# ali-vilab/VGen

Measured on AMD Instinct MI355X. Metric: denoise_steps_per_sec, higher is better.
Workload: dtype fp16

## Files before the change

include/vgen_hip.h:

```cpp
#ifndef VGEN_HIP_H
#define VGEN_HIP_H

#include <stddef.h>
#include <stdint.h>

#ifdef __cplusplus
extern "C" {
#endif

#define VGEN_ABI_VERSION 7

enum { VGEN_BF16 = 0, VGEN_F16 = 1, VGEN_F32 = 2 };

enum {
  VGEN_E_BADARG = -1,
  VGEN_E_UNSUPPORTED = -2,
  VGEN_E_WORKSPACE = -3
};

int vgen_version(void);
const char* vgen_last_error(void);

size_t vgen_groupnorm_ws_bytes(int64_t nb, int64_t S);
int vgen_groupnorm(const float* x1, int32_t C1, const float* x2, int32_t C2,
                   int64_t nb, int64_t S, int32_t groups, float eps,
                   const float* gamma, const float* beta, int32_t silu,
                   void* y, void* raw, int32_t raw_split, int32_t dtype,
                   float* ws, size_t ws_bytes, void* stream);

int vgen_groupnorm_cs(const float* x1, int32_t C1, const float* cs1,
                      const float* x2, int32_t C2, const float* cs2,
                      int64_t nb, int64_t S, int32_t groups, float eps,
                      const float* gamma, const float* beta, int32_t silu,
                      void* y, void* raw, int32_t raw_split, int32_t dtype,
                      float* ws, size_t ws_bytes, void* stream);

int vgen_embed_tokens(const int64_t* tokens, int64_t rows, int32_t L, int32_t d, int32_t vocab,
                      const float* table, const float* pos, float* out, void* stream);

int vgen_layernorm(const float* x, int64_t M, int32_t d, float eps,
                   const float* gamma, const float* beta,
                   void* y, int32_t dtype, void* stream);

enum { VGEN_TAP_LINEAR = 0, VGEN_TAP_CONV3X3 = 1, VGEN_TAP_TEMPORAL3 = 2 };
enum { VGEN_EPI_NONE = 0, VGEN_EPI_GEGLU = 1 };

typedef struct vgen_tapgemm_args {
  int64_t M;
  int32_t N;
  int32_t dtype;
  const void* A;
  int64_t lda;
  int32_t C1;
  int32_t taps;
  int32_t mode;
  int32_t Hi, Wi, Ho, Wo, stride, pad_t, pad_l, ups;
  int32_t F;
  int64_t S;
  const void* A2;
  int64_t lda2;
  int32_t C2;
  const void* W;
  int64_t ldw;
  const float* bias;
  const float* rowbias;
  int64_t rowbias_ld;
  int64_t rows_per_rb;
  const float* residual;
  int64_t ldr;
  void* out;
  int64_t ldo;
  int32_t out_dtype;
  int32_t epilogue;
  void* ws;
  size_t ws_bytes;
  int32_t crop_t;
  float* colstats;
  int32_t dualw;
  int32_t split_out;
} vgen_tapgemm_args;

size_t vgen_tapgemm_ws_bytes(const vgen_tapgemm_args* args);
int vgen_tapgemm(const vgen_tapgemm_args* args, void* stream);

int vgen_tapgemm_query_plan(const vgen_tapgemm_args* args, int32_t* out3);
int vgen_tapgemm_set_plans(const int64_t* rows, int32_t n);

typedef struct vgen_attn_args {
  const void* q;
  const void* k;
  const void* v;
  void* out;
  int32_t dtype;
  int32_t heads;
  int32_t nq, nk;
  int64_t nbatch;
  int64_t inner;
  int64_t q_rs, q_bo, q_bi;
  int64_t k_rs, k_bo, k_bi;
  int64_t v_rs, v_bo, v_bi;
  int64_t o_rs, o_bo, o_bi;
  float scale;
  int32_t causal;
} vgen_attn_args;

int vgen_attention(const vgen_attn_args* args, void* stream);

int vgen_attention_d80(const vgen_attn_args* args, void* stream);

int vgen_softmax_rows(const float* S, int64_t rows, int32_t cols, int64_t lds, float scale,
                      void* P, int64_t ldp, int32_t dtype, void* stream);


int vgen_act_cast(const float* x, void* y, int64_t n, int32_t act, int32_t dtype, void* stream);

int vgen_cast_split(const float* x, int64_t M, int32_t C, int64_t ldx, void* out, int64_t ldo, int32_t lo_off,
                    int32_t dtype, void* stream);

int vgen_timestep_embedding(const float* t, int32_t B, int32_t dim, void* out, int32_t dtype,
                            void* stream);

int vgen_linear_f32(const float* x, int32_t n, int32_t K, const float* W, const float* bias, int32_t N,
                    int32_t act_in, const float* add, float* out, void* stream);

int vgen_im2col3x3_small(const float* src, int64_t nimg, int32_t Fi, int32_t Cin, int32_t H,
                         int32_t W, int64_t s_bo, int64_t s_fi, int64_t s_c, int64_t s_y,
                         int64_t s_x, void* out, int32_t Kpad, int32_t dtype, int32_t split, void* stream);

int vgen_pointwise_small(const float* src, int64_t nimg, int32_t Fi, int32_t Cin, int32_t H,
                         int32_t W, int64_t s_bo, int64_t s_fi, int64_t s_c, int64_t s_y,
                         int64_t s_x, const float* Wm, const float* b, int32_t Cout, float* dst,
                         int64_t d_bo, int64_t d_fi, int64_t d_c, int64_t d_y, int64_t d_x,
                         void* stream);

int vgen_cfg_ddim_step(const float* xt, const float* y, const float* u, const float* noise,
                       const float* coef, float guide, int32_t use_guide, int32_t mean_type,
                       int64_t B, int64_t per_b, float* xt_1, float* x0_out, void* stream);

int vgen_cfg_ddim_step_units(const float* xt, int64_t xt_bstride, const float* y, const float* u,
                             const float* noise, const float* coef, const int64_t* t_idx, float guide,
                             int32_t use_guide, int32_t mean_type, int64_t B, int64_t per_b, float* xt_1,
                             float* x0_out, float* rep, int32_t nrep, int64_t rep_gstride,
                             int64_t rep_bstride, void* stream);

int vgen_gaussian_sample(const float* moments, const float* noise, int64_t nimg, int32_t zc,
                         int64_t HW, float scale, float* z, void* stream);

int vgen_lowfreq_filter(const float* x, int64_t nimg, int32_t H, int32_t W, int32_t C, float scale,
                        float* y, float* ws, size_t ws_bytes, void* stream);
int vgen_scale_channels(float* x, int64_t M, int32_t C, int32_t c0, int32_t c1, float s, void* stream);

int vgen_patchify(const float* x, int64_t B, int32_t C, int32_t H, int32_t W, int32_t P, int32_t Kpad, int32_t cls,
                  void* out, int32_t dtype, void* stream);

int vgen_conv3x3_small(const float* x, int64_t n, int32_t Cin, int32_t H, int32_t W, const float* w,
                       const float* b, int32_t Cout, int32_t stride, int32_t act, float* y, void* stream);
int vgen_adaptive_avgpool2d(const float* x, int64_t planes, int32_t H, int32_t W, int32_t Ho, int32_t Wo,
                            float* y, void* stream);
int vgen_frame_transformer(const float* x, int64_t B, int32_t F, int32_t d, int64_t HW, int32_t heads,
                           int32_t dim_head, int32_t hidden, const float* ln_w, const float* ln_b,
                           const float* wqkv, const float* wout, const float* bout, const float* w1,
                           const float* b1, const float* w2, const float* b2, float* y, int32_t last,
                           float out_scale, int32_t accumulate, void* stream);

int vgen_frames_u8(const float* x, int64_t rows, int32_t C, int64_t ldx, const float* mean,
                   const float* stdv, void* out, void* stream);

int vgen_adapter(const float* x, int64_t ldx, int64_t M, int32_t d, int32_t h, int32_t hp, const void* Wd,
                 const void* Wu, const float* bu, const float* hb, int64_t ldhb, int64_t rows_per_hb, float* out,
// ... 22 lines not shown
```

vgen_amd/build.py:

```python
from __future__ import annotations

import os
import shutil
import subprocess
import sys
from concurrent.futures import ThreadPoolExecutor

HERE = os.path.dirname(os.path.abspath(__file__))
CSRC = os.path.join(HERE, "csrc")
OBJ = os.path.join(CSRC, "_obj")
LIB = os.path.join(HERE, "libvgen_hip.so")
SOURCES = ["cabi.cpp", "tapgemm.hip", "panelgemm.hip", "norms.hip", "attention.hip", "misc.hip", "stems.hip", "adapter.hip"]
HEADERS = [os.path.join(CSRC, "common.h"), os.path.join(CSRC, "tapgemm_plans.inc"),
           os.path.join(HERE, "..", "include", "vgen_hip.h")]
FLAGS = ["--offload-arch=gfx950", "-O3", "-std=c++17", "-fPIC", "-Wall", "-Wno-unused-function", "-Wno-inline-asm",
         "-x", "hip"]


def _hipcc() -> str:
    for cand in (os.environ.get("HIPCC"), shutil.which("hipcc"), "/opt/rocm/bin/hipcc"):
        if cand and os.path.exists(cand):
            return cand
    raise RuntimeError("hipcc not found (need ROCm to build libvgen_hip.so)")


def _stale(target: str, deps) -> bool:
    if not os.path.exists(target):
        return True
    t = os.path.getmtime(target)
    return any(os.path.getmtime(d) > t for d in deps)


TUNING_LIB = os.path.join(HERE, "libvgen_hip_tuning.so")
HOST_LIB = os.path.join(HERE, "libvgen_host.so")
HOST_FLAGS = ["-O3", "-std=c++17", "-fPIC", "-shared", "-ffp-contract=off", "-Wall", "-pthread"]
HOST_ARCH = (["-march=x86-64-v3"], ["-mavx2", "-mf16c"])


def build_host(force: bool = False, verbose: bool = False) -> str:
    src = os.path.join(CSRC, "host_round.cpp")
    if force or _stale(HOST_LIB, [src]):
        gxx = os.environ.get("CXX") or shutil.which("g++") or shutil.which("c++")
        if not gxx:
            raise RuntimeError("g++ not found (need a host C++ compiler to build libvgen_host.so)")
        err = None
        for arch in HOST_ARCH:
            cmd = [gxx] + HOST_FLAGS + arch + [src, "-o", HOST_LIB]
            if verbose:
                print(" ".join(cmd), flush=True)
            r = subprocess.run(cmd, capture_output=True, text=True)
            if r.returncode == 0:
                err = None
                break
            err = "build failed: %s\n%s\n%s" % (" ".join(cmd), r.stdout, r.stderr)
        if err:
            raise RuntimeError(err)
    return HOST_LIB


def build_host_optional(force: bool = False, verbose: bool = False):
    try:
        return build_host(force=force, verbose=verbose)
    except (RuntimeError, OSError) as exc:
        import warnings
        warnings.warn(f"libvgen_host.so not built ({str(exc).splitlines()[0]}); vgen_amd.calibrate uses its torch loop")
        return None


def build(force: bool = False, verbose: bool = False, tuning: bool = False, variant: str = "", defines=()) -> str:
    if tuning:
        variant, defines = "tuning", tuple(defines) + ("VGEN_TUNING",)
    obj_dir = OBJ + ("_" + variant if variant else "")
    lib_path = os.path.join(HERE, f"libvgen_hip_{variant}.so") if variant else LIB
    flags = FLAGS + ["-D" + d for d in defines]
    os.makedirs(obj_dir, exist_ok=True)
    hipcc = _hipcc()
    jobs = []
    objs = []
    for src in SOURCES:
        s = os.path.join(CSRC, src)
        o = os.path.join(obj_dir, os.path.splitext(src)[0] + ".o")
        objs.append(o)
        if force or _stale(o, [s] + HEADERS):
            jobs.append([hipcc] + flags + ["-c", s, "-o", o])

    def run(cmd):
        if verbose:
            print(" ".join(cmd), flush=True)
        r = subprocess.run(cmd, capture_output=True, text=True)
        if r.returncode != 0:
            raise RuntimeError("build failed: %s\n%s\n%s" % (" ".join(cmd), r.stdout, r.stderr))
        return r

    if jobs:
        with ThreadPoolExecutor(max_workers=min(len(jobs), os.cpu_count() or 2)) as ex:
# ... 12 lines not shown
```

vgen_amd/csrc/tapgemm.hip:

```cpp
#include "common.h"
#include <stdio.h>
#include <stdlib.h>
#include <type_traits>

int vgen_panel_bn(const vgen_tapgemm_args& a);
int vgen_panel_launch(const vgen_tapgemm_args& a, hipStream_t s);

namespace {

struct RowState {
  int base;
  int a;
  int b;
};

constexpr int INVALID = -(1 << 24);

constexpr int ZERO_BYTES = 262144;
__device__ __attribute__((aligned(128))) unsigned char g_zeros[ZERO_BYTES];

typedef const __attribute__((address_space(1))) void* gptr_t;
typedef __attribute__((address_space(3))) void* lptr_t;


__device__ __forceinline__ void glds16(const void* src, unsigned char* lds_wave_base) {
  __builtin_amdgcn_global_load_lds((gptr_t)src, (lptr_t)lds_wave_base, 16, 0, 0);
}


template <int N>
__device__ __forceinline__ void wait_vmcnt() {
  asm volatile("s_waitcnt vmcnt(%0)" ::"n"(N) : "memory");
}

template <int CPR>
__device__ __forceinline__ int swz_key(int row) {
  if constexpr (CPR == 8) {
    return row & 7;
  } else {
    const int q = (row >> 2) & 3;
    return (4 - q) & 3;
  }
}

#ifdef VGEN_TUNING
#define VGEN_ABLATE_ARG(x) (x)
#else
#define VGEN_ABLATE_ARG(x) 0
#endif

template <typename T, int BM, int BN, int BK, int WM, int WN, int STAGES, bool PP, bool DW>
__global__ __launch_bounds__(WM* WN * 64, (WM * WN == 4) ? 2 : 1) void tapgemm_kernel(
    const vgen_tapgemm_args p, const int splitk, float* __restrict__ ws, const int ablate_arg, const int stagger,
    const int first_round) {
  static_assert(!PP || (WM * WN == 8 && STAGES == 3), "ping-pong needs 8 waves and a 3-stage ring");
  static_assert(!DW || (PP && BK == 64), "dual-W K-steps are built on the ping-pong schedule, 64-element K-tiles");
  const int ablate = VGEN_ABLATE_ARG(ablate_arg);
  constexpr int WPA = DW ? 2 : 1;
  constexpr int NT = WM * WN * 64;
  constexpr int ROW_BYTES = BK * 2;
  constexpr int CPR = ROW_BYTES / 16;
  constexpr int RPI = 64 / CPR;
  constexpr int RPP = NT / CPR;
  constexpr int KS = BK / 32;
  constexpr int WTM = BM / WM, WTN = BN / WN;
  constexpr int MF = WTM / 16, NF = WTN / 16;
  constexpr int RA = BM / RPP;
  constexpr int RBF = BN / RPP;
  constexpr int RBT = BN % RPP;
  constexpr int STAGE_BYTES = (BM + BN) * ROW_BYTES;
  constexpr int LPT = RA + RBF;
  static_assert(BM % RPP == 0 && RBT % RPI == 0, "tile rows must split into whole DMA instructions");

  extern __shared__ __attribute__((aligned(16))) unsigned char smem[];

  const int tid = threadIdx.x;
  const int lane = tid & 63;
  const int wave = __builtin_amdgcn_readfirstlane(tid >> 6);
  const int wm = wave / WN;
  const int wn = wave % WN;
  const int lr = lane & 15;
  const int lq = lane >> 4;
  const bool w_tail = RBT > 0 && wave * RPI < RBT;

  if (stagger > 0 && (int)(blockIdx.x + gridDim.x * blockIdx.y) < first_round && wave == 0) {
    const unsigned hw = __builtin_amdgcn_s_getreg((3 << 11) | ((WM * WN == 8 ? 8 : 0) << 6) | 4);
    if (hw & 1u)
      for (int i = 0; i < stagger; ++i) __builtin_amdgcn_s_sleep(16);
  }
// ... 792 lines not shown
    splitk = 1;
#ifdef VGEN_TUNING
  const char* ab = getenv("VGEN_TAPGEMM_ABLATE");
  const int ablate = ab ? atoi(ab) : 0;
#else
  const int ablate = 0;
#endif
  constexpr int BPC = (WM * WN == 4) ? 2 : 1;
  const int cus = vgen_device_cus();
  int stagger = 0;
  {
    int pct = BPC == 1 ? STAGGER_PCT_PP : STAGGER_PCT_DUAL, min_rounds = STAGGER_MIN_ROUNDS;
#ifdef VGEN_TUNING
    if (const char* e = getenv("VGEN_TAPGEMM_STAGGER")) {
      int a1 = 0, a2 = 0, a3 = min_rounds;
      if (sscanf(e, "%d,%d,%d", &a1, &a2, &a3) >= 2) {
        pct = BPC == 1 ? a1 : a2;
        min_rounds = a3;
      }
    }
#endif
    const int64_t blocks = grid * splitk;
    const double rounds = (double)blocks / ((double)cus * BPC);
    if (pct > 0 && rounds >= (double)min_rounds) {
      const int KT = a.taps * (a.C1 / 64) + a.C2 / 64;
      const int kts = (KT + splitk - 1) / splitk;
      const double tile_us = kts * (a.dualw ? 1.6 : 1.0) * (BM == 256 ? (BPC == 1 ? 0.0060 * BN : 0.0150 * BN) : 0.0050 * BN) + 7.0;
      stagger = (int)(tile_us * pct / 100.0 * 2400.0 / 1024.0 + 0.5);
    }
  }
  hipLaunchKernelGGL((tapgemm_kernel<T, BM, BN, BK, WM, WN, STAGES, PP, DW>), dim3((unsigned)grid, (unsigned)splitk),
                     dim3(WM * WN * 64), lds, stream, a, splitk, (float*)a.ws, ablate, stagger, cus * BPC);
  int rc = vgen_check_launch("tapgemm");
  if (rc || splitk == 1) return rc;
  const int n_out = a.epilogue == VGEN_EPI_GEGLU ? a.N / 2 : a.N;
  const int64_t threads = a.M * (n_out / 4);
  hipLaunchKernelGGL((splitk_reduce_kernel<T>), dim3((unsigned)((threads + 255) / 256)), dim3(256), 0,
                     stream, a, splitk, (const float*)a.ws);
  return vgen_check_launch("tapgemm(splitk reduce)");
}

int panel_bn(const vgen_tapgemm_args& a) {
#ifdef VGEN_TUNING
  if (env_int("VGEN_TAPGEMM_PANEL", 1) == 0) return 0;
#endif
  return vgen_panel_bn(a);
}

Plan full_plan(const vgen_tapgemm_args& a) {
  bool tabled = false;
  const Plan pl = make_plan(a, &tabled);
  if (!tabled)
    if (const int bn = panel_bn(a)) return Plan{SHAPE_PANEL, bn, 1};
  return pl;
}

template <typename T>
int dispatch(const vgen_tapgemm_args& a, hipStream_t s) {
  const Plan pl = full_plan(a);
  if (pl.shape == SHAPE_PANEL) return vgen_panel_launch(a, s);
  if (a.dualw) {
    if (pl.shape == SHAPE_PP128) {
      switch (pl.bn) {
        case 128: return launch<T, 128, 128, 64, 4, 2, 3, true, true>(a, pl.splitk, s);
        case 160: return launch<T, 128, 160, 64, 4, 2, 3, true, true>(a, pl.splitk, s);
        default: return launch<T, 128, 64, 64, 4, 2, 3, true, true>(a, pl.splitk, s);
      }
    }
    switch (pl.bn) {
      case 128: return launch<T, 256, 128, 64, 4, 2, 3, true, true>(a, pl.splitk, s);
      case 160: return launch<T, 256, 160, 64, 4, 2, 3, true, true>(a, pl.splitk, s);
      default: return launch<T, 256, 64, 64, 4, 2, 3, true, true>(a, pl.splitk, s);
    }
  }
  if (pl.shape == SHAPE_PP256) return launch<T, 256, 256, 32, 4, 2, 3, true>(a, pl.splitk, s);
  if (pl.shape == SHAPE_Q128) {
    switch (pl.bn) {
      case 128: return launch<T, 128, 128, 32, 2, 2, 3, false>(a, pl.splitk, s);
      case 160: return launch<T, 128, 160, 32, 2, 2, 3, false>(a, pl.splitk, s);
      default: return launch<T, 128, 64, 32, 2, 2, 3, false>(a, pl.splitk, s);
    }
  }
  if (pl.shape == SHAPE_PP) {
    switch (pl.bn) {
      case 128: return launch<T, 256, 128, 64, 4, 2, 3, true>(a, pl.splitk, s);
      case 160: return launch<T, 256, 160, 64, 4, 2, 3, true>(a, pl.splitk, s);
      default: return launch<T, 256, 64, 64, 4, 2, 3, true>(a, pl.splitk, s);
    }
  }
  if (pl.shape == SHAPE_PP128) {
    switch (pl.bn) {
      case 128: return launch<T, 128, 128, 64, 4, 2, 3, true>(a, pl.splitk, s);
      case 160: return launch<T, 128, 160, 64, 4, 2, 3, true>(a, pl.splitk, s);
      default: return launch<T, 128, 64, 64, 4, 2, 3, true>(a, pl.splitk, s);
    }
  }
  switch (pl.bn) {
    case 128: return launch<T, 256, 128, 32, 2, 2, 3, false>(a, pl.splitk, s);
    case 160: return launch<T, 256, 160, 32, 2, 2, 3, false>(a, pl.splitk, s);
    default: return launch<T, 256, 64, 32, 2, 2, 3, false>(a, pl.splitk, s);
  }
}

}

extern "C" int vgen_tapgemm_query_plan(const vgen_tapgemm_args* args, int32_t* out3) {
  if (!args || !out3 || args->N <= 0 || args->M <= 0 || args->C1 <= 0 || args->C1 % 64 || args->C2 % 64) return VGEN_E_BADARG;
  const Plan pl = full_plan(*args);
  out3[0] = pl.shape;
  out3[1] = pl.bn;
  out3[2] = pl.splitk;
  return 0;
}

extern "C" int vgen_tapgemm_set_plans(const int64_t* rows, int32_t n) {
  if (n < 0) {
    free(g_plans);
    g_plans = nullptr;
    g_nplans = -1;
    return 0;
  }
  if (n > 0 && !rows) return VGEN_E_BADARG;
  PlanEntry* t = (PlanEntry*)malloc(sizeof(PlanEntry) * (n > 0 ? n : 1));
  if (!t) return VGEN_E_BADARG;
  for (int i = 0; i < n; ++i) {
    const int64_t* r = rows + 12 * i;
    t[i] = PlanEntry{(int)r[0], r[1], (int)r[2], (int)r[3], (int)r[4], (int)r[5], (int)r[6], (int)r[7], (int)r[8],
                     (int)r[9], (int)r[10], (int)r[11]};
  }
  free(g_plans);
  g_plans = t;
  g_nplans = n;
  return 0;
}

extern "C" size_t vgen_tapgemm_ws_bytes(const vgen_tapgemm_args* args) {
  if (!args || args->N <= 0 || args->M <= 0 || args->C1 <= 0 || args->C1 % 64 || args->C2 % 64) return 0;
  const int s = full_plan(*args).splitk;
  return s > 1 ? (size_t)s * args->M * args->N * sizeof(float) : 0;
}

extern "C" int vgen_tapgemm(const vgen_tapgemm_args* args, void* stream) {
  if (!args) {
    vgen_set_error("tapgemm: null args");
    return VGEN_E_BADARG;
  }
  const vgen_tapgemm_args& a = *args;
  VGEN_REQUIRE(a.dtype == VGEN_BF16 || a.dtype == VGEN_F16, "tapgemm: dtype must be bf16/f16");
  VGEN_REQUIRE(a.M >= 0 && a.N > 0, "tapgemm: bad M/N");
  VGEN_REQUIRE(a.C1 > 0 && a.C1 % 64 == 0 && a.C2 >= 0 && a.C2 % 64 == 0,
               "tapgemm: C1=%d / C2=%d must be multiples of 64", a.C1, a.C2);
  VGEN_REQUIRE(a.dualw == 0 || a.dualw == 1, "tapgemm: dualw must be 0 or 1");
  VGEN_REQUIRE(a.lda % 8 == 0 && (a.C2 == 0 || a.lda2 % 8 == 0) && a.ldw % 8 == 0 &&
                   (a.ldw == 0 || a.ldw >= ((int64_t)a.taps * a.C1 + a.C2) * (a.dualw ? 2 : 1)),
               "tapgemm: lda/lda2/ldw must be multiples of 8 (ldw >= K, 2 K with dualw)");
  VGEN_REQUIRE(vgen_aligned16(a.A) && vgen_aligned16(a.W) && vgen_aligned16(a.out) &&
                   (a.C2 == 0 || (a.A2 && vgen_aligned16(a.A2))),
               "tapgemm: pointers must be 16-byte aligned");
  VGEN_REQUIRE(a.bias == nullptr || vgen_aligned16(a.bias), "tapgemm: bias alignment");
  VGEN_REQUIRE(a.residual == nullptr || vgen_aligned16(a.residual), "tapgemm: residual alignment");
  VGEN_REQUIRE(a.rowbias == nullptr || (vgen_aligned16(a.rowbias) && a.rows_per_rb > 0),
               "tapgemm: rowbias alignment / rows_per_rb");
  VGEN_REQUIRE(a.out_dtype == VGEN_F32 || a.out_dtype == a.dtype, "tapgemm: out_dtype");
  VGEN_REQUIRE(a.ws == nullptr || vgen_aligned16(a.ws), "tapgemm: workspace alignment");
  switch (a.mode) {
    case VGEN_TAP_LINEAR:
      VGEN_REQUIRE(a.taps == 1, "tapgemm: linear mode needs taps == 1");
      break;
    case VGEN_TAP_CONV3X3:
      VGEN_REQUIRE(a.taps == 9 && a.Hi > 0 && a.Wi > 0 && a.Ho > 0 && a.Wo > 0 &&
                       (a.stride == 1 || a.stride == 2) && (a.ups == 0 || a.ups == 1) && a.crop_t >= 0 &&
                       (a.crop_t == 0 || a.ups == 1),
                   "tapgemm: bad conv3x3 geometry");
      VGEN_REQUIRE(a.M % ((int64_t)a.Ho * a.Wo) == 0, "tapgemm: M not a multiple of Ho*Wo");
      VGEN_REQUIRE((a.M / ((int64_t)a.Ho * a.Wo)) * a.Hi * a.Wi < (1LL << 31),
                   "tapgemm: source row index overflows int32");
      break;
    case VGEN_TAP_TEMPORAL3:
      VGEN_REQUIRE(a.taps == 3 && a.F > 0 && a.S > 0 && a.M % (a.S * a.F) == 0,
                   "tapgemm: bad temporal geometry");
      break;
    default:
      vgen_set_error("tapgemm: unknown mode %d", a.mode);
      return VGEN_E_BADARG;
  }
  VGEN_REQUIRE(a.M + 256 < (1LL << 31), "tapgemm: M overflows int32 row index");
  VGEN_REQUIRE(a.lda >= 0 && a.lda < (1LL << 30) && a.lda2 >= 0 && a.lda2 < (1LL << 30),
               "tapgemm: lda / lda2 must be in [0, 2^30)");
  VGEN_REQUIRE(((int64_t)a.taps * a.C1 + a.C2) * (a.dualw ? 4 : 2) <= ZERO_BYTES - 128,
               "tapgemm: K = %lld too long (<= 131008; <= 65504 with dualw)",
               (long long)((int64_t)a.taps * a.C1 + a.C2));
  if (a.epilogue == VGEN_EPI_GEGLU) {
    VGEN_REQUIRE(a.N % 64 == 0 && a.rowbias == nullptr && (a.ldo % 4 == 0) &&
                     (a.residual == nullptr || a.ldr % 4 == 0),
                 "tapgemm: GEGLU needs N %% 64 == 0, no rowbias, ldo/ldr %% 4 == 0");
// ... 21 lines not shown
```

vgen_amd/lib.py:

```python
from __future__ import annotations

import ctypes as C
import os

HERE = os.path.dirname(os.path.abspath(__file__))
LIB_PATH = os.environ.get("VGEN_HIP_LIB") or os.path.join(HERE, "libvgen_hip.so")

VGEN_BF16, VGEN_F16, VGEN_F32 = 0, 1, 2
TAP_LINEAR, TAP_CONV3X3, TAP_TEMPORAL3 = 0, 1, 2
EPI_NONE, EPI_GEGLU = 0, 1
ABI_VERSION = 7


class VgenHipError(RuntimeError):
    pass


class TapGemmArgs(C.Structure):
    _fields_ = [
        ("M", C.c_int64), ("N", C.c_int32), ("dtype", C.c_int32),
        ("A", C.c_void_p), ("lda", C.c_int64), ("C1", C.c_int32), ("taps", C.c_int32),
        ("mode", C.c_int32),
        ("Hi", C.c_int32), ("Wi", C.c_int32), ("Ho", C.c_int32), ("Wo", C.c_int32),
        ("stride", C.c_int32), ("pad_t", C.c_int32), ("pad_l", C.c_int32), ("ups", C.c_int32),
        ("F", C.c_int32), ("S", C.c_int64),
        ("A2", C.c_void_p), ("lda2", C.c_int64), ("C2", C.c_int32),
        ("W", C.c_void_p), ("ldw", C.c_int64),
        ("bias", C.c_void_p), ("rowbias", C.c_void_p), ("rowbias_ld", C.c_int64),
        ("rows_per_rb", C.c_int64), ("residual", C.c_void_p), ("ldr", C.c_int64),
        ("out", C.c_void_p), ("ldo", C.c_int64), ("out_dtype", C.c_int32),
        ("epilogue", C.c_int32),
        ("ws", C.c_void_p), ("ws_bytes", C.c_size_t), ("crop_t", C.c_int32),
        ("colstats", C.c_void_p), ("dualw", C.c_int32), ("split_out", C.c_int32),
    ]


class AttnArgs(C.Structure):
    _fields_ = [
        ("q", C.c_void_p), ("k", C.c_void_p), ("v", C.c_void_p), ("out", C.c_void_p),
        ("dtype", C.c_int32), ("heads", C.c_int32), ("nq", C.c_int32), ("nk", C.c_int32),
        ("nbatch", C.c_int64), ("inner", C.c_int64),
        ("q_rs", C.c_int64), ("q_bo", C.c_int64), ("q_bi", C.c_int64),
        ("k_rs", C.c_int64), ("k_bo", C.c_int64), ("k_bi", C.c_int64),
        ("v_rs", C.c_int64), ("v_bo", C.c_int64), ("v_bi", C.c_int64),
        ("o_rs", C.c_int64), ("o_bo", C.c_int64), ("o_bi", C.c_int64),
        ("scale", C.c_float), ("causal", C.c_int32),
    ]


_i32, _i64, _f32, _vp, _sz = C.c_int32, C.c_int64, C.c_float, C.c_void_p, C.c_size_t
SYMBOLS = {
    "vgen_version": (C.c_int, []),
    "vgen_last_error": (C.c_char_p, []),
    "vgen_groupnorm_ws_bytes": (_sz, [_i64, _i64]),
    "vgen_groupnorm": (C.c_int, [_vp, _i32, _vp, _i32, _i64, _i64, _i32, _f32, _vp, _vp, _i32,
                                 _vp, _vp, _i32, _i32, _vp, _sz, _vp]),
    "vgen_groupnorm_cs": (C.c_int, [_vp, _i32, _vp, _vp, _i32, _vp, _i64, _i64, _i32, _f32, _vp, _vp, _i32,
                                    _vp, _vp, _i32, _i32, _vp, _sz, _vp]),
    "vgen_layernorm": (C.c_int, [_vp, _i64, _i32, _f32, _vp, _vp, _vp, _i32, _vp]),
    "vgen_tapgemm_ws_bytes": (_sz, [C.POINTER(TapGemmArgs)]),
    "vgen_tapgemm": (C.c_int, [C.POINTER(TapGemmArgs), _vp]),
    "vgen_tapgemm_query_plan": (C.c_int, [C.POINTER(TapGemmArgs), _vp]),
    "vgen_tapgemm_set_plans": (C.c_int, [_vp, _i32]),
    "vgen_attention": (C.c_int, [C.POINTER(AttnArgs), _vp]),
    "vgen_attention_d80": (C.c_int, [C.POINTER(AttnArgs), _vp]),
    "vgen_softmax_rows": (C.c_int, [_vp, _i64, _i32, _i64, _f32, _vp, _i64, _i32, _vp]),
    "vgen_act_cast": (C.c_int, [_vp, _vp, _i64, _i32, _i32, _vp]),
    "vgen_cast_split": (C.c_int, [_vp, _i64, _i32, _i64, _vp, _i64, _i32, _i32, _vp]),
    "vgen_timestep_embedding": (C.c_int, [_vp, _i32, _i32, _vp, _i32, _vp]),
    "vgen_conv3x3_small": (C.c_int, [_vp, _i64, _i32, _i32, _i32, _vp, _vp, _i32, _i32, _i32, _vp, _vp]),
    "vgen_patchify": (C.c_int, [_vp, _i64, _i32, _i32, _i32, _i32, _i32, _i32, _vp, _i32, _vp]),
    "vgen_adaptive_avgpool2d": (C.c_int, [_vp, _i64, _i32, _i32, _i32, _i32, _vp, _vp]),
    "vgen_frame_transformer": (C.c_int, [_vp, _i64, _i32, _i32, _i64, _i32, _i32, _i32, _vp, _vp, _vp, _vp, _vp, _vp,
                                         _vp, _vp, _vp, _vp, _i32, _f32, _i32, _vp]),
    "vgen_embed_tokens": (C.c_int, [_vp, _i64, _i32, _i32, _i32, _vp, _vp, _vp, _vp]),
    "vgen_linear_f32": (C.c_int, [_vp, _i32, _i32, _vp, _vp, _i32, _i32, _vp, _vp, _vp]),
    "vgen_im2col3x3_small": (C.c_int, [_vp, _i64, _i32, _i32, _i32, _i32, _i64, _i64, _i64, _i64,
                                       _i64, _vp, _i32, _i32, _i32, _vp]),
    "vgen_pointwise_small": (C.c_int, [_vp, _i64, _i32, _i32, _i32, _i32, _i64, _i64, _i64, _i64,
                                       _i64, _vp, _vp, _i32, _vp, _i64, _i64, _i64, _i64, _i64,
                                       _vp]),
    "vgen_cfg_ddim_step_units": (C.c_int, [_vp, _i64, _vp, _vp, _vp, _vp, _vp, _f32, _i32, _i32, _i64, _i64, _vp,
                                           _vp, _vp, _i32, _i64, _i64, _vp]),
    "vgen_cfg_ddim_step": (C.c_int, [_vp, _vp, _vp, _vp, _vp, _f32, _i32, _i32, _i64, _i64, _vp,
                                     _vp, _vp]),
    "vgen_gaussian_sample": (C.c_int, [_vp, _vp, _i64, _i32, _i64, _f32, _vp, _vp]),
    "vgen_lowfreq_filter": (C.c_int, [_vp, _i64, _i32, _i32, _i32, _f32, _vp, _vp, _sz, _vp]),
    "vgen_scale_channels": (C.c_int, [_vp, _i64, _i32, _i32, _i32, _f32, _vp]),
    "vgen_frames_u8": (C.c_int, [_vp, _i64, _i32, _i64, _vp, _vp, _vp, _vp]),
    "vgen_cfg_stats_ws_bytes": (_sz, [_i64]),
    "vgen_cfg_stats": (C.c_int, [_vp, _vp, _f32, _i32, _i64, _i64, _vp, _vp, _sz, _vp]),
    "vgen_gauss_x0": (C.c_int, [_vp, _vp, _vp, _f32, _vp, _i32, _i64, _i64, _vp, _vp, _vp]),
    "vgen_lincomb4": (C.c_int, [_vp, _vp, _vp, _vp, _f32, _f32, _f32, _f32, _vp, _i64, _vp]),
    "vgen_repeat_rows": (C.c_int, [_vp, _i64, _i32, _vp, _vp]),
    "vgen_gather_rows_f32": (C.c_int, [_vp, _i64, _i64, _vp, _i64, _vp, _vp]),
    "vgen_adapter": (C.c_int, [_vp, _i64, _i64, _i32, _i32, _i32, _vp, _vp, _vp, _vp, _i64, _i64, _vp, _i64, _i32, _vp]),
    "vgen_dpmpp2m_sde_step": (C.c_int, [_vp, _vp, _vp, _vp, _f32, _f32, _f32, _f32, _f32, _f32, _vp, _i64, _vp]),
}

_lib = None


def load(path: str | None = None):
    global _lib
    if _lib is not None and path is None:
        return _lib
    p = path or LIB_PATH
    import torch
    if not os.path.exists(p):
        raise VgenHipError(
            f"{p} not found: build it with `python -m vgen_amd.build` (hipcc, gfx950). "
            "There is no CPU fallback for the hot path.")
    try:
        lib = C.CDLL(p)
    except OSError as e:
        raise VgenHipError(f"cannot load {p}: {e}") from e
    for name, (res, args) in SYMBOLS.items():
        try:
            fn = getattr(lib, name)
        except AttributeError as e:
            raise VgenHipError(f"{p} does not export {name}") from e
        fn.restype = res
        fn.argtypes = args
    v = lib.vgen_version()
    if v != ABI_VERSION:
        raise VgenHipError(f"ABI version mismatch: library {v}, binding {ABI_VERSION}")
    _lib = lib
    return lib


def check(rc: int, what: str):
    if rc != 0:
        msg = _lib.vgen_last_error().decode("utf-8", "replace") if _lib is not None else "?"
        raise VgenHipError(f"{what} failed (rc={rc}): {msg}")
```

Baseline: 33.78.

## Add persistent tap-GEMM kernel for 256-row PP tiles with cross-tile prefetch

Adds a persistent variant of the PP-shape tap GEMM. It launches one workgroup per CU, walks tiles in XCD-aware contiguous runs, and prefetches the next tile's first K-slices while the current tile finishes, so the pipeline stays full across tile boundaries. It also uses direct global-to-LDS loads with swizzling and staggers waves on odd SEs. This is meant to remove per-tile launch and pipeline fill/drain bubbles and tail imbalance, at the cost of a large new hand-scheduled kernel with timing heuristics such as a stagger formula.

Result: no change. 33.56 (-0.7%).

```diff
diff --git a/include/vgen_hip.h b/include/vgen_hip.h
--- a/include/vgen_hip.h
+++ b/include/vgen_hip.h
@@ -85,6 +85,7 @@
 
 int vgen_tapgemm_query_plan(const vgen_tapgemm_args* args, int32_t* out3);
 int vgen_tapgemm_set_plans(const int64_t* rows, int32_t n);
+int vgen_tapgemm_is_persistent(const vgen_tapgemm_args* args);
 
 typedef struct vgen_attn_args {
   const void* q;
diff --git a/vgen_amd/build.py b/vgen_amd/build.py
--- a/vgen_amd/build.py
+++ b/vgen_amd/build.py
@@ -10,7 +10,7 @@
 CSRC = os.path.join(HERE, "csrc")
 OBJ = os.path.join(CSRC, "_obj")
 LIB = os.path.join(HERE, "libvgen_hip.so")
-SOURCES = ["cabi.cpp", "tapgemm.hip", "panelgemm.hip", "norms.hip", "attention.hip", "misc.hip", "stems.hip", "adapter.hip"]
+SOURCES = ["cabi.cpp", "tapgemm.hip", "tapgemm_persist.hip", "panelgemm.hip", "norms.hip", "attention.hip", "misc.hip", "stems.hip", "adapter.hip"]
 HEADERS = [os.path.join(CSRC, "common.h"), os.path.join(CSRC, "tapgemm_plans.inc"),
            os.path.join(HERE, "..", "include", "vgen_hip.h")]
 FLAGS = ["--offload-arch=gfx950", "-O3", "-std=c++17", "-fPIC", "-Wall", "-Wno-unused-function", "-Wno-inline-asm",
diff --git a/vgen_amd/csrc/tapgemm.hip b/vgen_amd/csrc/tapgemm.hip
--- a/vgen_amd/csrc/tapgemm.hip
+++ b/vgen_amd/csrc/tapgemm.hip
@@ -5,6 +5,8 @@
 
 int vgen_panel_bn(const vgen_tapgemm_args& a);
 int vgen_panel_launch(const vgen_tapgemm_args& a, hipStream_t s);
+int vgen_pp_persist_ok(const vgen_tapgemm_args& a, int bn);
+int vgen_pp_persist_launch(const vgen_tapgemm_args& a, int bn, hipStream_t s);
 
 namespace {
 
@@ -963,6 +965,7 @@
     }
   }
   if (pl.shape == SHAPE_PP) {
+    if (pl.splitk == 1 && vgen_pp_persist_ok(a, pl.bn)) return vgen_pp_persist_launch(a, pl.bn, s);
     switch (pl.bn) {
       case 128: return launch<T, 256, 128, 64, 4, 2, 3, true>(a, pl.splitk, s);
       case 160: return launch<T, 256, 160, 64, 4, 2, 3, true>(a, pl.splitk, s);
@@ -992,6 +995,12 @@
   out3[1] = pl.bn;
   out3[2] = pl.splitk;
   return 0;
+}
+
+extern "C" int vgen_tapgemm_is_persistent(const vgen_tapgemm_args* args) {
+  if (!args || args->N <= 0 || args->M <= 0 || args->C1 <= 0 || args->C1 % 64 || args->C2 % 64) return VGEN_E_BADARG;
+  const Plan pl = full_plan(*args);
+  return pl.shape == SHAPE_PP && pl.splitk == 1 && !args->dualw && vgen_pp_persist_ok(*args, pl.bn) ? 1 : 0;
 }
 
 extern "C" int vgen_tapgemm_set_plans(const int64_t* rows, int32_t n) {
diff --git a/vgen_amd/csrc/tapgemm_persist.hip b/vgen_amd/csrc/tapgemm_persist.hip
--- /dev/null
+++ b/vgen_amd/csrc/tapgemm_persist.hip
@@ -0,0 +1,538 @@
+#include "common.h"
+#include <stdio.h>
+#include <stdlib.h>
+#include <type_traits>
+
+namespace {
+
+struct RowState {
+  int base;
+  int a;
+  int b;
+};
+
+constexpr int INVALID = -(1 << 24);
+
+constexpr int ZERO_BYTES = 262144;
+__device__ __attribute__((aligned(128))) unsigned char g_pzeros[ZERO_BYTES];
+
+typedef const __attribute__((address_space(1))) void* gptr_t;
+typedef __attribute__((address_space(3))) void* lptr_t;
+
+__device__ __forceinline__ void glds16(const void* src, unsigned char* lds_wave_base) {
+  __builtin_amdgcn_global_load_lds((gptr_t)src, (lptr_t)lds_wave_base, 16, 0, 0);
+}
+
+template <int N>
+__device__ __forceinline__ void wait_vmcnt() {
+  asm volatile("s_waitcnt vmcnt(%0)" ::"n"(N) : "memory");
+}
+
+__device__ __forceinline__ int swz_key8(int row) { return row & 7; }
+
+template <typename T, int BN, bool ESYNC>
+__global__ __launch_bounds__(512, 1) void tapgemm_persist_kernel(const vgen_tapgemm_args p, const int ntiles, const int stagger) {
+  constexpr int BM = 256, BK = 64, WN = 2, STAGES = 3;
+  constexpr int NT = 512;
+  constexpr int ROW_BYTES = BK * 2;
+  constexpr int CPR = ROW_BYTES / 16;
+  constexpr int RPI = 64 / CPR;
+  constexpr int RPP = NT / CPR;
+  constexpr int KS = BK / 32;
+  constexpr int WTM = 64, WTN = BN / WN;
+  constexpr int MF = WTM / 16, NF = WTN / 16;
+  constexpr int RA = BM / RPP;
+  constexpr int RBF = BN / RPP;
+  constexpr int RBT = BN % RPP;
+  constexpr int STAGE_BYTES = (BM + BN) * ROW_BYTES;
+  constexpr int LPT = RA + RBF;
+  constexpr int NP = LPT + (RBT > 0 ? 1 : 0);
+  static_assert(RBT % RPI == 0, "tile rows must split into whole DMA instructions");
+
+  extern __shared__ __attribute__((aligned(16))) unsigned char smem[];
+
+  const int tid = threadIdx.x;
+  const int lane = tid & 63;
+  const int wave = __builtin_amdgcn_readfirstlane(tid >> 6);
+  const int wm = wave / WN;
+  const int wn = wave % WN;
+  const int lr = lane & 15;
+  const int lq = lane >> 4;
+  const bool w_tail = RBT > 0 && wave * RPI < RBT;
+
+  if (stagger > 0 && wave == 0) {
+    const unsigned hw = __builtin_amdgcn_s_getreg((3 << 11) | (8 << 6) | 4);
+    if (hw & 1u)
+      for (int i = 0; i < stagger; ++i) __builtin_amdgcn_s_sleep(16);
+  }
+
+  const int tiles_n = (p.N + BN - 1) / BN;
+  unsigned run0, my_n, nbx;
+  const unsigned lb = blockIdx.x >> 3;
+  {
+    const unsigned G = gridDim.x, xcd = blockIdx.x & 7u;
+    const unsigned q = (unsigned)ntiles >> 3, r = (unsigned)ntiles & 7u;
+    run0 = xcd < r ? xcd * (q + 1) : r * (q + 1) + (xcd - r) * q;
+    const unsigned runlen = q + (xcd < r ? 1u : 0u);
+    nbx = (G >> 3) + (xcd < (G & 7u) ? 1u : 0u);
+    my_n = lb < runlen ? (runlen - lb + nbx - 1) / nbx : 0u;
+  }
+  if (my_n == 0) return;
+
+  const uint16_t* __restrict__ A = (const uint16_t*)p.A;
+  const uint16_t* __restrict__ A2 = (const uint16_t*)p.A2;
+  const uint16_t* __restrict__ W = (const uint16_t*)p.W;
+  const int64_t ldw = p.ldw ? p.ldw : ((int64_t)p.taps * p.C1 + p.C2);
+
+  const int ld_c = tid % CPR;
+  const int ld_r = tid / CPR;
+
+  const int cpt1 = p.C1 / BK;
+  const int T1 = p.taps * cpt1;
+  const int KT = T1 + p.C2 / BK;
+
+  RowState rs[RA];
+  unsigned mvalid = 0;
+  const char* pc[NP];
+  const char* const zline = (const char*)g_pzeros;
+  const int src_cb = (ld_c ^ swz_key8(ld_r)) * 16;
+  const int wave_row0 = wave * RPI;
+  const char* const zl = zline + src_cb;
+  const unsigned lda_b = (unsigned)p.lda * 2u, lda2_b = (unsigned)p.lda2 * 2u;
+  int kt_next = KT - 1;
+  int left = 0;
+  unsigned is_j = ~0u;
+  unsigned lm0 = 0;
+
+  auto gather_a = [&](int kt) __attribute__((always_inline)) {
+    if (kt < T1) {
+      const int tap = kt / cpt1;
+      const int cch = kt - tap * cpt1;
+      left = cpt1 - cch;
+      const char* const a_cb = (const char*)A + (cch * BK * 2 + src_cb);
+      if (p.mode == VGEN_TAP_CONV3X3) {
+        const int d0 = tap / 3, d1 = tap - 3 * d0;
+        const unsigned Hv = (unsigned)((p.Hi << p.ups) - 2 * p.crop_t), Wv = (unsigned)(p.Wi << p.ups);
+#pragma unroll
+        for (int i = 0; i < RA; ++i) {
+          const int iy = rs[i].a + d0, ix = rs[i].b + d1;
+          const bool ok = ((unsigned)iy < Hv) & ((unsigned)ix < Wv);
+          const unsigned row = (unsigned)rs[i].base + (unsigned)((iy + p.crop_t) >> p.ups) * (unsigned)p.Wi + (unsigned)(ix >> p.ups);
+          const char* const real = a_cb + (uint64_t)row * lda_b;
+          pc[i] = ok ? real : zl;
+        }
+      } else if (p.mode == VGEN_TAP_TEMPORAL3) {
+        const int dt_ = tap - 1;
+#pragma unroll
+        for (int i = 0; i < RA; ++i) {
+          const bool ok = (unsigned)(rs[i].a + dt_) < (unsigned)p.F;
+          const unsigned row = (unsigned)(rs[i].base + dt_ * p.S);
+          const char* const real = a_cb + (uint64_t)row * lda_b;
+          pc[i] = ok ? real : zl;
+        }
+      } else {
+#pragma unroll
+        for (int i = 0; i < RA; ++i) {
+          const bool ok = rs[i].base >= 0;
+          const char* const real = a_cb + (uint64_t)(unsigned)rs[i].base * lda_b;
+          pc[i] = ok ? real : zl;
+        }
+      }
+    } else {
+      left = KT - kt + 1;
+      const char* const a_cb = (const char*)A2 + ((kt - T1) * BK * 2 + src_cb);
+#pragma unroll
+      for (int i = 0; i < RA; ++i) {
+        const bool ok = (mvalid >> i) & 1u;
+        const char* const real = a_cb + (uint64_t)(lm0 + ld_r + RPP * i) * lda2_b;
+        pc[i] = ok ? real : zl;
+      }
+    }
+  };
+  auto setup_tile = [&](unsigned j) __attribute__((always_inline)) {
+    kt_next = 0;
+    if (j >= my_n) {
+#pragma unroll
+      for (int i = 0; i < NP; ++i) pc[i] = zl;
+      left = 1 << 30;
+      return;
+    }
+    const unsigned tile = run0 + lb + j * nbx;
+    lm0 = (tile / (unsigned)tiles_n) * BM;
+    const int ln0 = (int)(tile % (unsigned)tiles_n) * BN;
+    mvalid = 0;
+#pragma unroll
+    for (int i = 0; i < RA; ++i) {
+      const unsigned m = lm0 + ld_r + RPP * i;
+      const bool ok = m < (unsigned)p.M;
+      if (ok) mvalid |= 1u << i;
+      if (p.mode == VGEN_TAP_CONV3X3) {
+        const unsigned hw = p.Ho * p.Wo;
+        const unsigned img = m / hw;
+        const unsigned rem = m - img * hw;
+        const unsigned oy = rem / (unsigned)p.Wo;
+        const unsigned ox = rem - oy * p.Wo;
+        rs[i].base = img * p.Hi * p.Wi;
+        rs[i].a = ok ? (int)oy * p.stride - p.pad_t : INVALID;
+        rs[i].b = (int)ox * p.stride - p.pad_l;
+      } else if (p.mode == VGEN_TAP_TEMPORAL3) {
+        const unsigned fs = m / (unsigned)p.S;
+        rs[i].base = (int)m;
+        rs[i].a = ok ? (int)(fs % (unsigned)p.F) : INVALID;
+        rs[i].b = 0;
+      } else {
+        rs[i].base = ok ? (int)m : -1;
+        rs[i].a = 0;
+        rs[i].b = 0;
+      }
+    }
+    gather_a(0);
+#pragma unroll
+    for (int i = 0; i < NP - RA; ++i) {
+      const int n = ln0 + ld_r + RPP * i;
+      const bool ok = n < p.N;
+      pc[RA + i] = (ok ? (const char*)(W + (int64_t)n * ldw) : zline) + src_cb;
+    }
+  };
+  auto advance = [&]() __attribute__((always_inline)) {
+    ++kt_next;
+    if (kt_next == KT) {
+      ++is_j;
+      setup_tile(is_j);
+    } else {
+      if (--left == 0) {
+        gather_a(kt_next);
+      } else {
+#pragma unroll
+        for (int i = 0; i < RA; ++i) pc[i] += ROW_BYTES;
+      }
+#pragma unroll
+      for (int i = RA; i < NP; ++i) pc[i] += ROW_BYTES;
+    }
+  };
+  auto piece_dst = [&](int stage, int j) __attribute__((always_inline)) -> unsigned char* {
+    unsigned char* const base = smem + stage * STAGE_BYTES + wave_row0 * ROW_BYTES;
+    return j < RA ? base + j * RPP * ROW_BYTES : base + (BM + (j - RA) * RPP) * ROW_BYTES;
+  };
+  auto dma = [&](int j, int stage) __attribute__((always_inline)) { glds16(pc[j], piece_dst(stage, j)); };
+
+  const bool geglu = p.epilogue == VGEN_EPI_GEGLU;
+  const int n_out = geglu ? p.N / 2 : p.N;
+  const bool res_folded = p.residual != nullptr && !geglu;
+  f32x4 acc[NF][MF];
+
+  const int rd_row = lr * ROW_BYTES;
+  const int sw = swz_key8(lr);
+  u32x4 wf[KS][NF], xf[KS][MF];
+
+  auto read_phase = [&](int stage, int stage_pf) __attribute__((always_inline)) {
+    const unsigned char* bw = smem + stage * STAGE_BYTES + BM * ROW_BYTES + wn * WTN * ROW_BYTES + rd_row;
+    const unsigned char* bx = smem + stage * STAGE_BYTES + (wm * WTM) * ROW_BYTES + rd_row;
+    constexpr int NRF = NF + MF;
+    constexpr int NR = KS * NRF;
+    constexpr int EVERY = (NR + NP) / (NP + 1) > 0 ? (NR + NP) / (NP + 1) : 1;
+    int piece = 0;
+#pragma unroll
+    for (int r = 0; r < NR; ++r) {
+      const int ks = r / NRF, q = r % NRF;
+      const int co = ((ks * 4 + lq) ^ sw) << 4;
+      if (q < NF) wf[ks][q] = *(const u32x4*)(bw + q * 16 * ROW_BYTES + co);
+      else xf[ks][q - NF] = *(const u32x4*)(bx + (q - NF) * 16 * ROW_BYTES + co);
+      if ((r % EVERY) == EVERY - 1 && piece < NP) {
+        __builtin_amdgcn_sched_barrier(0);
+        if (piece < LPT) {
+          dma(piece, stage_pf);
+        } else if (RBT > 0 && w_tail) {
+          dma(NP - 1, stage_pf);
+        }
+        ++piece;
+        __builtin_amdgcn_sched_barrier(0);
+      }
+    }
+#pragma unroll
+    for (int j = 0; j < NP; ++j)
+      if (j >= piece) {
+        if (j < LPT) {
+          dma(j, stage_pf);
+        } else if (RBT > 0 && w_tail) {
+          dma(NP - 1, stage_pf);
+        }
+      }
+  };
+  auto mfma_phase = [&]() __attribute__((always_inline)) {
+#pragma unroll
+    for (int ks = 0; ks < KS; ++ks)
+#pragma unroll
+      for (int ni = 0; ni < NF; ++ni)
+#pragma unroll
+        for (int mi = 0; mi < MF; ++mi) acc[ni][mi] = T::mfma32(wf[ks][ni], xf[ks][mi], acc[ni][mi]);
+  };
+
+  auto epilogue = [&](const int64_t m0, const int n0) __attribute__((always_inline)) {
+    float* const of = (float*)p.out;
+    uint16_t* const oh = (uint16_t*)p.out;
+    f32x4 bv[NF];
+#pragma unroll
+    for (int ni = 0; ni < NF; ++ni) {
+      const int n = n0 + wn * WTN + ni * 16 + lq * 4;
+      bv[ni] = (p.bias && n < p.N) ? *(const f32x4*)(p.bias + n) : f32x4{0.f, 0.f, 0.f, 0.f};
+    }
+    if (p.out_dtype != VGEN_F32 && (p.ldo & 7) == 0 && (!geglu || NF % 4 == 0)) {
+#pragma unroll
+      for (int mi = 0; mi < MF; ++mi) {
+        __builtin_amdgcn_sched_barrier(0);
+        const int64_t m = m0 + wm * WTM + mi * 16 + lr;
+        if (m >= p.M) continue;
+        const float* rbp = p.rowbias ? p.rowbias + (m / p.rows_per_rb) * p.rowbias_ld : nullptr;
+        auto store_pair16 = [&](int frag0_col, bool pair_ok, const f32x4& va, const f32x4& vb, int64_t m_) __attribute__((always_inline)) {
+          u32x2 pa = pack4<T>(va.x, va.y, va.z, va.w);
+          u32x2 pb = pack4<T>(vb.x, vb.y, vb.z, vb.w);
+          if (pair_ok) {
+            const auto sx = __builtin_amdgcn_permlane16_swap(pa.x, pb.x, false, false);
+            const auto sy = __builtin_amdgcn_permlane16_swap(pa.y, pb.y, false, false);
+            const u32x4 q = {sx[0], sy[0], sx[1], sy[1]};
+            *(u32x4*)(oh + m_ * p.ldo + frag0_col + (lq & 1) * 16 + (lq >> 1) * 8) = q;
+          } else {
+            if (frag0_col + lq * 4 < n_out) *(u32x2*)(oh + m_ * p.ldo + frag0_col + lq * 4) = pa;
+            if (frag0_col + 16 + lq * 4 < n_out) *(u32x2*)(oh + m_ * p.ldo + frag0_col + 16 + lq * 4) = pb;
+          }
+        };
+        if (!geglu) {
+          auto final_val = [&](int ni) __attribute__((always_inline)) -> f32x4 {
+            const int n = n0 + wn * WTN + ni * 16 + lq * 4;
+            f32x4 v = acc[ni][mi];
+            if (n < p.N) {
+              v += bv[ni];
+              if (rbp) v += *(const f32x4*)(rbp + n);
+            }
+            return v;
+          };
+          auto lo_of = [&](const f32x4& v) __attribute__((always_inline)) -> f32x4 {
+            const u32x2 h = pack4<T>(v.x, v.y, v.z, v.w);
+            return f32x4{v.x - T::to_f32((uint16_t)(h.x & 0xffffu)), v.y - T::to_f32((uint16_t)(h.x >> 16)),
+                         v.z - T::to_f32((uint16_t)(h.y & 0xffffu)), v.w - T::to_f32((uint16_t)(h.y >> 16))};
+          };
+#pragma unroll
+          for (int ni = 0; ni + 1 < NF; ni += 2) {
+            const int c0 = n0 + wn * WTN + ni * 16;
+            const f32x4 va = final_val(ni), vb = final_val(ni + 1);
+            store_pair16(c0, c0 + 32 <= p.N, va, vb, m);
+            if (p.split_out) store_pair16(p.N + c0, c0 + 32 <= p.N, lo_of(va), lo_of(vb), m);
+          }
+          if constexpr (NF % 2 == 1) {
+            const int n = n0 + wn * WTN + (NF - 1) * 16 + lq * 4;
+            if (n < p.N) {
+              const f32x4 v = final_val(NF - 1);
+              *(u32x2*)(oh + m * p.ldo + n) = pack4<T>(v.x, v.y, v.z, v.w);
+              if (p.split_out) {
+                const f32x4 l = lo_of(v);
+                *(u32x2*)(oh + m * p.ldo + p.N + n) = pack4<T>(l.x, l.y, l.z, l.w);
+              }
+            }
+          }
+        } else if constexpr (NF % 4 == 0) {
+          auto gated = [&](int np) __attribute__((always_inline)) -> f32x4 {
+            const int pn = n0 + wn * WTN + np * 32 + lq * 4;
+            const int j = (n0 + wn * WTN) / 2 + np * 16 + lq * 4;
+            f32x4 o = {0.f, 0.f, 0.f, 0.f};
+            if (pn < p.N) {
+              const f32x4 val = acc[2 * np][mi] + bv[2 * np];
+              const f32x4 gat = acc[2 * np + 1][mi] + bv[2 * np + 1];
+              o = geglu4(val, gat);
+              if (p.residual) o += *(const f32x4*)(p.residual + m * p.ldr + j);
+            }
+            return o;
+          };
+#pragma unroll
+          for (int np = 0; np < NF / 2; np += 2) {
+            const int j0 = (n0 + wn * WTN) / 2 + np * 16;
+            store_pair16(j0, j0 + 32 <= n_out, gated(np), gated(np + 1), m);
+          }
+        }
+      }
+      return;
+    }
+#pragma unroll
+    for (int mi = 0; mi < MF; ++mi) {
+      __builtin_amdgcn_sched_barrier(0);
+      const int64_t m = m0 + wm * WTM + mi * 16 + lr;
+      if (m >= p.M) continue;
+      const float* rbp = p.rowbias ? p.rowbias + (m / p.rows_per_rb) * p.rowbias_ld : nullptr;
+      if (!geglu) {
+#pragma unroll
+        for (int ni = 0; ni < NF; ++ni) {
+          const int n = n0 + wn * WTN + ni * 16 + lq * 4;
+          if (n >= p.N) continue;
+          f32x4 v = acc[ni][mi];
+          v += bv[ni];
+          if (rbp) v += *(const f32x4*)(rbp + n);
+          if (p.out_dtype == VGEN_F32) {
+            *(f32x4*)(of + m * p.ldo + n) = v;
+          } else {
+            *(u32x2*)(oh + m * p.ldo + n) = pack4<T>(v.x, v.y, v.z, v.w);
+          }
+        }
+      } else if constexpr (NF % 2 == 0) {
+#pragma unroll
+        for (int np = 0; np < NF / 2; ++np) {
+          const int pn = n0 + wn * WTN + np * 32 + lq * 4;
+          if (pn >= p.N) continue;
+          const int j = (n0 + wn * WTN) / 2 + np * 16 + lq * 4;
+          const f32x4 val = acc[2 * np][mi] + bv[2 * np];
+          const f32x4 gat = acc[2 * np + 1][mi] + bv[2 * np + 1];
+          f32x4 o = geglu4(val, gat);
+          if (p.residual) o += *(const f32x4*)(p.residual + m * p.ldr + j);
+          if (p.out_dtype == VGEN_F32) {
+            *(f32x4*)(of + m * p.ldo + j) = o;
+          } else {
+            *(u32x2*)(oh + m * p.ldo + j) = pack4<T>(o.x, o.y, o.z, o.w);
+          }
+        }
+      }
+    }
+  };
+
+#pragma nounroll
+  for (int i = 0; i < STAGES; ++i) {
+    if (i > 0) {
+#pragma unroll
+      for (int j = 0; j < LPT; ++j) dma(j, i - 1);
+      if (RBT > 0 && w_tail) dma(NP - 1, i - 1);
+    }
+    advance();
+  }
+  int st_c = 0, st_l = STAGES - 1;
+  auto wait_next = [&]() __attribute__((always_inline)) {
+    if (w_tail) wait_vmcnt<LPT + 1>();
+    else wait_vmcnt<LPT>();
+  };
+  const bool follower = wave >= 4;
+  wait_next();
+  __builtin_amdgcn_s_barrier();
+  if (follower) __builtin_amdgcn_s_barrier();
+  asm volatile("" ::: "memory");
+
+  for (unsigned cj = 0; cj < my_n; ++cj) {
+    const unsigned tile = run0 + lb + cj * nbx;
+    const int64_t m0 = (int64_t)(tile / (unsigned)tiles_n) * BM;
+    const int n0 = (int)(tile % (unsigned)tiles_n) * BN;
+#pragma unroll
+    for (int ni = 0; ni < NF; ++ni)
+#pragma unroll
+      for (int mi = 0; mi < MF; ++mi) acc[ni][mi] = f32x4{0.f, 0.f, 0.f, 0.f};
+    if (res_folded) {
+#pragma unroll
+      for (int mi = 0; mi < MF; ++mi) {
+        const int64_t m = m0 + wm * WTM + mi * 16 + lr;
+#pragma unroll
+        for (int ni = 0; ni < NF; ++ni) {
+          const int n = n0 + wn * WTN + ni * 16 + lq * 4;
+          if (m < p.M && n < p.N) acc[ni][mi] = *(const f32x4*)(p.residual + m * p.ldr + n);
+        }
+      }
+    }
+    __builtin_amdgcn_sched_barrier(0);
+    read_phase(st_c, st_l);
+    wait_next();
+#pragma unroll
+    for (int ni = 0; ni < NF; ++ni)
+#pragma unroll
+      for (int mi = 0; mi < MF; ++mi) asm volatile("" : "+v"(acc[ni][mi]));
+    for (int k = 0;;) {
+      asm volatile("s_waitcnt lgkmcnt(0)" ::: "memory");
+      __builtin_amdgcn_s_barrier();
+      __builtin_amdgcn_sched_barrier(0);
+      mfma_phase();
+      __builtin_amdgcn_sched_barrier(0);
+      advance();
+      __builtin_amdgcn_s_barrier();
+      asm volatile("" ::: "memory");
+      st_c = st_c == STAGES - 1 ? 0 : st_c + 1;
+      st_l = st_l == STAGES - 1 ? 0 : st_l + 1;
+      if (++k == KT) break;
+      read_phase(st_c, st_l);
+      wait_next();
+    }
+    __builtin_amdgcn_sched_barrier(0);
+    if constexpr (ESYNC) {
+      if (!follower) __builtin_amdgcn_s_barrier();
+      asm volatile("" ::: "memory");
+    }
+    epilogue(m0, n0);
+    if constexpr (ESYNC) {
+      if (follower) __builtin_amdgcn_s_barrier();
+      asm volatile("" ::: "memory");
+    }
+    __builtin_amdgcn_sched_barrier(0);
+  }
+  if (!follower) __builtin_amdgcn_s_barrier();
+  wait_vmcnt<0>();
+}
+
+template <typename T, int BN, bool ESYNC>
+int launch_persist(const vgen_tapgemm_args& a, hipStream_t stream) {
+  constexpr size_t lds = (size_t)3 * (256 + BN) * 64 * 2;
+  static bool attr_done[VGEN_MAX_DEVICES] = {false};
+  const int dev = vgen_device_slot();
+  if (!attr_done[dev]) {
+    hipError_t e = hipFuncSetAttribute((const void*)tapgemm_persist_kernel<T, BN, ESYNC>, hipFuncAttributeMaxDynamicSharedMemorySize,
+                                       (int)lds);
+    if (e != hipSuccess) {
+      vgen_set_error("tapgemm(persistent): hipFuncSetAttribute(%zu B LDS) failed: %s", lds, hipGetErrorString(e));
+      return (int)e;
+    }
+    attr_done[dev] = true;
+  }
+  const int cus = vgen_device_cus();
+  const int64_t tiles = ((a.M + 255) / 256) * ((a.N + BN - 1) / BN);
+  int stagger = 0;
+  if ((double)tiles / (double)cus >= 2.0) {
+    const int KT = a.taps * (a.C1 / 64) + a.C2 / 64;
+    const double tile_us = KT * 0.0060 * BN + 7.0;
+    stagger = (int)(tile_us * 50 / 100.0 * 2400.0 / 1024.0 + 0.5);
+  }
+  hipLaunchKernelGGL((tapgemm_persist_kernel<T, BN, ESYNC>), dim3((unsigned)cus), dim3(512), lds, stream, a, (int)tiles, stagger);
+  return vgen_check_launch("tapgemm(persistent)");
+}
+
+template <typename T>
+int persist_dispatch(const vgen_tapgemm_args& a, int bn, hipStream_t s) {
+#ifdef VGEN_TUNING
+  if (const char* e = getenv("VGEN_TAPGEMM_PERSIST"))
+    if (atoi(e) == 2) switch (bn) {
+        case 128: return launch_persist<T, 128, true>(a, s);
+        case 160: return launch_persist<T, 160, true>(a, s);
+        case 64: return launch_persist<T, 64, true>(a, s);
+      }
+#endif
+  switch (bn) {
+    case 128: return launch_persist<T, 128, false>(a, s);
+    case 160: return launch_persist<T, 160, false>(a, s);
+    case 64: return launch_persist<T, 64, false>(a, s);
+  }
+  vgen_set_error("tapgemm(persistent): no %d-column instantiation", bn);
+  return VGEN_E_BADARG;
+}
+
+}
+
+int vgen_pp_persist_ok(const vgen_tapgemm_args& a, int bn) {
+#ifdef VGEN_TUNING
+  if (const char* e = getenv("VGEN_TAPGEMM_PERSIST"))
+    if (atoi(e) == 0) return 0;
+#endif
+  if (bn != 128 && bn != 160 && bn != 64) return 0;
+  if (a.dualw || a.colstats) return 0;
+  const bool geglu = a.epilogue == VGEN_EPI_GEGLU;
+  const int n_out = geglu ? a.N / 2 : a.N;
+  const bool vec = ((n_out & 3) == 0) && ((a.ldo & 3) == 0) && (a.residual == nullptr || (a.ldr & 3) == 0) &&
+                   (a.rowbias == nullptr || (a.rowbias_ld & 3) == 0);
+  if (!vec || (geglu && bn == 160)) return 0;
+  const int cus = vgen_device_cus();
+  const int64_t tiles = ((a.M + 255) / 256) * ((a.N + bn - 1) / bn);
+  return cus >= 8 && tiles > cus && tiles <= 0x7fffffffLL;
+}
+
+int vgen_pp_persist_launch(const vgen_tapgemm_args& a, int bn, hipStream_t s) {
+  return a.dtype == VGEN_BF16 ? persist_dispatch<BF16>(a, bn, s) : persist_dispatch<F16>(a, bn, s);
+}
diff --git a/vgen_amd/lib.py b/vgen_amd/lib.py
--- a/vgen_amd/lib.py
+++ b/vgen_amd/lib.py
@@ -61,6 +61,7 @@
     "vgen_tapgemm_ws_bytes": (_sz, [C.POINTER(TapGemmArgs)]),
     "vgen_tapgemm": (C.c_int, [C.POINTER(TapGemmArgs), _vp]),
     "vgen_tapgemm_query_plan": (C.c_int, [C.POINTER(TapGemmArgs), _vp]),
+    "vgen_tapgemm_is_persistent": (C.c_int, [C.POINTER(TapGemmArgs)]),
     "vgen_tapgemm_set_plans": (C.c_int, [_vp, _i32]),
     "vgen_attention": (C.c_int, [C.POINTER(AttnArgs), _vp]),
     "vgen_attention_d80": (C.c_int, [C.POINTER(AttnArgs), _vp]),
```
